# mfouda/epsilon

Measured on AMD Instinct MI355X. Metric: ADMM iters/sec, dense Lasso 1e4x5e4, higher is better.
Workload: dtype f32

## Files before the change

epsilon_amd/csrc/kernels_factor.hip:

```cpp
#include <hip/hip_runtime.h>

#include <algorithm>
#include <cstdlib>
#include <type_traits>

#include "kernels.h"
#include "options.h"

namespace eps {
namespace k {

namespace {

constexpr int NB = 64;

template <int L> __device__ inline float ReadLane(float v) {
  return __builtin_bit_cast(float, __builtin_amdgcn_readlane(__builtin_bit_cast(int, v), L));
}
template <int L> __device__ inline double ReadLane(double v) {
  const long long b = __builtin_bit_cast(long long, v);
  const int lo = __builtin_amdgcn_readlane(static_cast<int>(b), L);
  const int hi = __builtin_amdgcn_readlane(static_cast<int>(b >> 32), L);
  return __builtin_bit_cast(double, (static_cast<long long>(hi) << 32) |
                                        static_cast<unsigned int>(lo));
}

template <int I, int N> struct StaticFor {
  template <class F> __device__ static inline void Run(F&& f) {
    f(std::integral_constant<int, I>());
    StaticFor<I + 1, N>::Run(f);
  }
};
template <int N> struct StaticFor<N, N> {
  template <class F> __device__ static inline void Run(F&&) {}
};

constexpr int KC = 32;

template <class T> __device__ inline void Pin(T& v) { asm volatile("" : "+v"(v)); }

template <class T> __device__ __forceinline__ bool CholRows(T (&r)[NB], int lane) {
  bool bad = false;
  StaticFor<0, NB>::Run([&](auto jj) {
    constexpr int j = decltype(jj)::value;
    T d = ReadLane<j>(r[j]);
    if (!(d > T(0))) {
      bad = true;
      d = T(1);
    }
    const T dj = sqrt(d);
    const T l = lane > j ? r[j] / dj : (lane == j ? dj : T(0));
    r[j] = l;
    StaticFor<0, (NB - 1 - j + 3) / 4>::Run([&](auto gg) {
      constexpr int c0 = j + 1 + 4 * decltype(gg)::value;
      T b[4];
      StaticFor<0, 4>::Run([&](auto ii) {
        constexpr int c = c0 + decltype(ii)::value;
        if constexpr (c < NB) b[decltype(ii)::value] = ReadLane<c>(l);
      });
      StaticFor<0, 4>::Run([&](auto ii) {
        constexpr int c = c0 + decltype(ii)::value;
        if constexpr (c < NB) r[c] -= l * b[decltype(ii)::value];
      });
      StaticFor<0, 4>::Run([&](auto ii) {
        constexpr int c = c0 + decltype(ii)::value;
        if constexpr (c < NB) Pin(r[c]);
      });
    });
  });
  return bad;
}

template <class T> __device__ __forceinline__ bool CholRowsSolve(T (&r)[NB], T (&t)[NB], int lane) {
  bool bad = false;
  StaticFor<0, NB>::Run([&](auto jj) {
    constexpr int j = decltype(jj)::value;
    T d = ReadLane<j>(r[j]);
    if (!(d > T(0))) {
      bad = true;
      d = T(1);
    }
    const T dj = sqrt(d);
    const T l = lane > j ? r[j] / dj : (lane == j ? dj : T(0));
    r[j] = l;
    const T x = t[j] / dj;
    t[j] = x;
    StaticFor<0, (NB - 1 - j + 3) / 4>::Run([&](auto gg) {
      constexpr int c0 = j + 1 + 4 * decltype(gg)::value;
      T b[4];
      StaticFor<0, 4>::Run([&](auto ii) {
        constexpr int c = c0 + decltype(ii)::value;
        if constexpr (c < NB) b[decltype(ii)::value] = ReadLane<c>(l);
      });
      StaticFor<0, 4>::Run([&](auto ii) {
        constexpr int c = c0 + decltype(ii)::value;
        if constexpr (c < NB) {
          r[c] -= l * b[decltype(ii)::value];
          t[c] -= x * b[decltype(ii)::value];
        }
      });
      StaticFor<0, 4>::Run([&](auto ii) {
        constexpr int c = c0 + decltype(ii)::value;
        if constexpr (c < NB) {
          Pin(r[c]);
          Pin(t[c]);
        }
      });
    });
  });
  return bad;
}

template <class T>
__global__ __launch_bounds__(256) void PotrfDiagStepKernel(T* W, int64_t ld, int64_t K0, int64_t k0,
                                                           int kb, int* flag) {
  __shared__ T D[NB][NB];
  __shared__ T Pc[KC][NB];
  const int t = threadIdx.x, r = t & 63, q = t >> 6;
  T acc[16];
#pragma unroll
  for (int c = 0; c < 16; ++c) {
    const int col = q * 16 + c;
    T v = (r == col) ? T(1) : T(0);
    if (r < kb && col < kb && r >= col) v = W[(k0 + r) + (k0 + col) * ld];
    acc[c] = v;
  }
  constexpr int PF = KC * NB / 256;
  T pf[PF];
  auto fetch = [&](int64_t kk) {
#pragma unroll
    for (int i = 0; i < PF; ++i) {
      const int idx = t + i * 256, rr = idx & 63, k = idx >> 6;
      pf[i] = rr < kb ? W[(k0 + rr) + (kk + k) * ld] : T(0);
    }
  };
  if (K0 < k0) fetch(K0);
  for (int64_t kk = K0; kk < k0; kk += KC) {
    __syncthreads();
#pragma unroll
    for (int i = 0; i < PF; ++i) {
      const int idx = t + i * 256;
      Pc[idx >> 6][idx & 63] = pf[i];
    }
    __syncthreads();
    if (kk + KC < k0) fetch(kk + KC);
#pragma unroll 4
    for (int k = 0; k < KC; ++k) {
      const T a = Pc[k][r];
#pragma unroll
      for (int c = 0; c < 16; ++c) acc[c] -= a * Pc[k][q * 16 + c];
    }
  }
#pragma unroll
  for (int c = 0; c < 16; ++c) D[q * 16 + c][r] = acc[c];
  __syncthreads();
  if (q != 0) return;
  T row[NB];
  StaticFor<0, NB>::Run([&](auto cc) {
    constexpr int c = decltype(cc)::value;
    row[c] = r >= c ? D[c][r] : T(0);
  });
  const bool bad = CholRows(row, r);
  if (bad && r == 0) *flag = 1;
  StaticFor<0, NB>::Run([&](auto cc) {
    constexpr int c = decltype(cc)::value;
    if (r < kb && c < kb && r >= c) W[(k0 + r) + (k0 + c) * ld] = row[c];
  });
}

template <class T>
__global__ __launch_bounds__(256) void PotrfPanelStepKernel(T* W, int64_t ld, int64_t n, int64_t K0,
                                                            int64_t k0, int kb) {
  __shared__ T Tt[NB][NB];
  __shared__ T buf[2 * KC * NB];
  T* Lr = buf;
  T* Pc = buf + KC * NB;
  const int t = threadIdx.x, r = t & 63, q = t >> 6;
  const int64_t row0 = k0 + kb + static_cast<int64_t>(blockIdx.x) * NB;
  const int64_t row = row0 + r;
  const bool live = row < n;
  T acc[16];
#pragma unroll
  for (int c = 0; c < 16; ++c) {
    const int col = q * 16 + c;
    acc[c] = (live && col < kb) ? W[row + (k0 + col) * ld] : T(0);
  }
  constexpr int PF = KC * NB / 256;
  T pfl[PF], pfp[PF];
  auto fetch = [&](int64_t kk) {
#pragma unroll
    for (int i = 0; i < PF; ++i) {
      const int idx = t + i * 256, rr = idx & 63, k = idx >> 6;
      pfl[i] = (row0 + rr < n) ? W[(row0 + rr) + (kk + k) * ld] : T(0);
      pfp[i] = rr < kb ? W[(k0 + rr) + (kk + k) * ld] : T(0);
    }
  };
  if (K0 < k0) fetch(K0);
  for (int64_t kk = K0; kk < k0; kk += KC) {
    __syncthreads();
#pragma unroll
    for (int i = 0; i < PF; ++i) {
      const int idx = t + i * 256;
      Lr[idx] = pfl[i];
      Pc[idx] = pfp[i];
    }
    __syncthreads();
    if (kk + KC < k0) fetch(kk + KC);
#pragma unroll 4
    for (int k = 0; k < KC; ++k) {
      const T a = Lr[k * NB + r];
#pragma unroll
      for (int c = 0; c < 16; ++c) acc[c] -= a * Pc[k * NB + q * 16 + c];
    }
  }
  __syncthreads();
#pragma unroll
  for (int c = 0; c < 16; ++c) Tt[q * 16 + c][r] = acc[c];
  for (int idx = t; idx < NB * NB; idx += 256) {
    const int j = idx & 63, k = idx >> 6;
    T v = (j == k) ? T(1) : T(0);
    if (j < kb && k < kb && j >= k) v = W[(k0 + j) + (k0 + k) * ld];
    buf[j * NB + k] = v;
  }
  __syncthreads();
  if (q == 0) {
#pragma unroll 1
    for (int jb = 0; jb < NB; jb += 8) {
      T tv[8];
#pragma unroll
      for (int jj = 0; jj < 8; ++jj) tv[jj] = Tt[jb + jj][r];
#pragma unroll 1
      for (int k8 = 0; k8 < jb; k8 += 8) {
#pragma unroll
        for (int kk = 0; kk < 8; ++kk) {
          const T xk = Tt[k8 + kk][r];
#pragma unroll
          for (int jj = 0; jj < 8; ++jj) tv[jj] -= xk * buf[(jb + jj) * NB + k8 + kk];
        }
      }
#pragma unroll
      for (int jj = 0; jj < 8; ++jj) {
#pragma unroll
        for (int kk = 0; kk < jj; ++kk) tv[jj] -= tv[kk] * buf[(jb + jj) * NB + jb + kk];
        tv[jj] /= buf[(jb + jj) * NB + jb + jj];
      }
#pragma unroll
      for (int jj = 0; jj < 8; ++jj) Tt[jb + jj][r] = tv[jj];
    }
  }
  __syncthreads();
  if (live) {
#pragma unroll
    for (int c = 0; c < 16; ++c) {
      const int col = q * 16 + c;
      if (col < kb) W[row + (k0 + col) * ld] = Tt[col][r];
    }
  }
}

__global__ __launch_bounds__(256) void PotrfFusedStepKernel(float* W, int64_t ld, int64_t n, int64_t K0,
                                                            int64_t k0, int kb, int* flag,
                                                            float* __restrict__ dfac) {
  using T = float;
  __shared__ T Tt[NB][NB];
  __shared__ T Dd[NB][NB];
  __shared__ T buf[2 * KC * NB];
  T* Lr = buf;
  T* Pc = buf + KC * NB;
  const int t = threadIdx.x, r = t & 63, q = t >> 6;
  const int64_t row0 = k0 + kb + static_cast<int64_t>(blockIdx.x) * NB;
  const int64_t row = row0 + r;
  const bool live = row < n;
  T acc[16], dac[16];
#pragma unroll
  for (int c = 0; c < 16; ++c) {
    const int col = q * 16 + c;
    acc[c] = (live && col < kb) ? W[row + (k0 + col) * ld] : T(0);
    T v = (r == col) ? T(1) : T(0);
    if (r < kb && col < kb && r >= col) v = W[(k0 + r) + (k0 + col) * ld];
    dac[c] = v;
  }
  constexpr int PF = KC * NB / 256;
  T pfl[PF], pfp[PF];
  auto fetch = [&](int64_t kk) {
#pragma unroll
    for (int i = 0; i < PF; ++i) {
      const int idx = t + i * 256, rr = idx & 63, k = idx >> 6;
      pfl[i] = (row0 + rr < n) ? W[(row0 + rr) + (kk + k) * ld] : T(0);
      pfp[i] = rr < kb ? W[(k0 + rr) + (kk + k) * ld] : T(0);
    }
  };
  if (K0 < k0) fetch(K0);
  for (int64_t kk = K0; kk < k0; kk += KC) {
    __syncthreads();
#pragma unroll
    for (int i = 0; i < PF; ++i) {
      const int idx = t + i * 256;
      Lr[idx] = pfl[i];
      Pc[idx] = pfp[i];
    }
    __syncthreads();
    if (kk + KC < k0) fetch(kk + KC);
#pragma unroll 4
    for (int k = 0; k < KC; ++k) {
      const T a = Lr[k * NB + r], d = Pc[k * NB + r];
#pragma unroll
      for (int c = 0; c < 16; ++c) {
        const T pc = Pc[k * NB + q * 16 + c];
        acc[c] -= a * pc;
        dac[c] -= d * pc;
      }
    }
  }
  __syncthreads();
#pragma unroll
  for (int c = 0; c < 16; ++c) {
    Tt[q * 16 + c][r] = acc[c];
    Dd[q * 16 + c][r] = dac[c];
  }
  __syncthreads();
  if (q == 0) {
    T rowv[NB], tv[NB];
    StaticFor<0, NB>::Run([&](auto cc) {
      constexpr int c = decltype(cc)::value;
      rowv[c] = r >= c ? Dd[c][r] : T(0);
      tv[c] = Tt[c][r];
    });
    const bool bad = CholRowsSolve(rowv, tv, r);
    if (bad && r == 0) *flag = 1;
    StaticFor<0, NB>::Run([&](auto cc) {
      constexpr int c = decltype(cc)::value;
      Tt[c][r] = tv[c];
      if (blockIdx.x == 0) dfac[c * NB + r] = rowv[c];
    });
  }
  __syncthreads();
  if (live) {
#pragma unroll
    for (int c = 0; c < 16; ++c) {
      const int col = q * 16 + c;
      if (col < kb) W[row + (k0 + col) * ld] = Tt[col][r];
    }
  }
}

template <class T>
__global__ __launch_bounds__(64) void TrtriDiagBlocksKernel(const T* W, int64_t ld, int64_t n, T* Dinv) {
  const int lane = threadIdx.x;
  const int64_t k0 = static_cast<int64_t>(blockIdx.x) * NB;
  const int kb = static_cast<int>(n - k0 < NB ? n - k0 : NB);
  T r[NB];
  StaticFor<0, NB>::Run([&](auto cc) {
    constexpr int c = decltype(cc)::value;
    T v = (lane == c) ? T(1) : T(0);
    if (lane < kb && c < kb && lane >= c) v = W[(k0 + lane) + (k0 + c) * ld];
    r[c] = v;
  });
  T x[NB];
  StaticFor<0, NB>::Run([&](auto ii) {
    constexpr int j = NB - 1 - decltype(ii)::value;
    const T ajj = T(1) / ReadLane<j>(r[j]);
    T acc = T(0);
    StaticFor<0, (NB - 1 - j + 3) / 4>::Run([&](auto gg) {
      constexpr int c0 = j + 1 + 4 * decltype(gg)::value;
      T b[4];
      StaticFor<0, 4>::Run([&](auto ii) {
        constexpr int kk = c0 + decltype(ii)::value;
        if constexpr (kk < NB) b[decltype(ii)::value] = ReadLane<kk>(r[j]);
      });
      StaticFor<0, 4>::Run([&](auto ii) {
        constexpr int kk = c0 + decltype(ii)::value;
        if constexpr (kk < NB) acc += x[kk] * b[decltype(ii)::value];
      });
      Pin(acc);
    });
    x[j] = lane > j ? -acc * ajj : (lane == j ? ajj : T(0));
  });
  T* out = Dinv + static_cast<int64_t>(blockIdx.x) * NB * NB;
  StaticFor<0, NB>::Run([&](auto cc) {
    constexpr int c = decltype(cc)::value;
    out[lane + c * NB] = (lane < kb && c < kb && lane >= c) ? x[c] : T(0);
  });
}

template <class T>
__global__ __launch_bounds__(256) void ScatterDiagBlocksKernel(const T* Dinv, T* X, int64_t ld, int64_t n) {
  const int64_t k0 = static_cast<int64_t>(blockIdx.x) * NB;
  const T* src = Dinv + static_cast<int64_t>(blockIdx.x) * NB * NB;
  for (int idx = threadIdx.x; idx < NB * NB; idx += 256) {
    const int r = idx & 63, c = idx >> 6;
    if (k0 + r < n && k0 + c < n) X[(k0 + r) + (k0 + c) * ld] = src[idx];
  }
}

DVec Sub(const DVec& W, int64_t i, int64_t j, int64_t ld) {
  const int64_t off = i + j * ld;
  return W.Slice(off, W.n - off);
}

}

namespace {
void PotrfBlocked(const DVec& W, int64_t n, const DVec& dinv, int* flag);
void CheckFlag(int* flag);
void DoublingInverse(const DVec& W, const DVec& X, int64_t n, const DVec& dinv, int64_t cap);
}

void SpdInverseInPlace(const DVec& W, int64_t n, DVec* factor_inverse) {
  EPS_CHECK(W.n >= n * n);
  if (n == 0) return;
  Runtime& rt = Runtime::Get();
  hipStream_t s = rt.stream();
  ProfScope prof("spd_inverse", n);
  const DType dt = W.dt;
  const int64_t ld = n;
  const int64_t nb = (n + NB - 1) / NB;

  DVec dinv = DVec::Empty(nb * NB * NB, dt);
  auto flag_buf = rt.Alloc(sizeof(int));
  int* flag = static_cast<int*>(flag_buf->p);
  EPS_HIP(hipMemsetAsync(flag, 0, sizeof(int), s));
  {
    ProfScope p1("potrf", n);
    PotrfBlocked(W, n, dinv, flag);
  }

  DVec X = DVec::Zeros(n * n, dt);
  {
    ProfScope p2("trtri", n);
    DoublingInverse(W, X, n, dinv, n);
  }
  ProfScope p3("lauum", n);

  if (!SyrkSplitF16LowerTriangular(n, X, ld, W, ld)) {
    const int64_t B = 1024;
    Fill(W.Slice(0, n * n), 0.0);
    for (int64_t p0 = 0; p0 < n; p0 += B) {
      const int64_t pb = std::min<int64_t>(B, n - p0);
      const int64_t cp = p0 + pb;
      DVec Xp = Sub(X, p0, 0, ld);
      Gemm(true, false, cp, cp, pb, 1.0, Xp, ld, Xp, ld, 1.0, W, ld, true);
    }
  }
  SymmetrizeFromLower(W, n, ld);

  CheckFlag(flag);
  if (factor_inverse) *factor_inverse = X;
}

namespace {

void CheckFlag(int* flag) {
  hipStream_t s = Runtime::Get().stream();
  int host_flag = 0;
  EPS_HIP(hipMemcpyAsync(&host_flag, flag, sizeof(int), hipMemcpyDeviceToHost, s));
  EPS_HIP(hipStreamSynchronize(s));
  EPS_CHECK_MSG(host_flag == 0, "dense inverse: matrix is not positive definite");
}

void DoublingInverse(const DVec& W, const DVec& X, int64_t n, const DVec& dinv, int64_t cap) {
  hipStream_t s = Runtime::Get().stream();
  const DType dt = W.dt;
  const int64_t ld = n;
  const int64_t nb = (n + NB - 1) / NB;
  if (dt == F32)
    hipLaunchKernelGGL(ScatterDiagBlocksKernel<float>, dim3(static_cast<unsigned>(nb)), dim3(256), 0, s,
                       dinv.as<float>(), X.as<float>(), ld, n);
  else
    hipLaunchKernelGGL(ScatterDiagBlocksKernel<double>, dim3(static_cast<unsigned>(nb)), dim3(256), 0, s,
                       dinv.as<double>(), X.as<double>(), ld, n);
  const int64_t half = std::min<int64_t>(cap, n) / 2 + NB;
  const int64_t kBatchBelow = 4096;
  DVec tmp2 = DVec::Empty(std::max<int64_t>({1, half * half, n * std::min(cap, kBatchBelow) / 4}), dt);
  for (int64_t sz = NB; sz < cap; sz *= 2) {
    int64_t r_first = 0;
    if (sz < kBatchBelow) {
      const int64_t P = n / (2 * sz);
      if (P > 0) {
        const int64_t stride = 2 * sz * (ld + 1);
        EPS_CHECK(tmp2.n >= P * sz * sz);
        GemmBatched(false, false, sz, sz, sz, 1.0, Sub(W, sz, 0, ld), ld, stride, X, ld, stride, 0.0,
                    tmp2, sz, sz * sz, P);
        GemmBatched(false, false, sz, sz, sz, -1.0, Sub(X, sz, sz, ld), ld, stride, tmp2, sz, sz * sz,
                    0.0, Sub(X, sz, 0, ld), ld, stride, P);
      }
      r_first = P * 2 * sz;
    }
    for (int64_t r0 = r_first; r0 + sz < n; r0 += 2 * sz) {
      const int64_t s1 = sz;
      const int64_t s2 = std::min<int64_t>(sz, n - (r0 + sz));
      DVec L21 = Sub(W, r0 + s1, r0, ld);
      DVec X11 = Sub(X, r0, r0, ld);
      DVec X22 = Sub(X, r0 + s1, r0 + s1, ld);
      DVec X21 = Sub(X, r0 + s1, r0, ld);
      EPS_CHECK(tmp2.n >= s2 * s1);
      DVec T = tmp2.Slice(0, s2 * s1);
      const int64_t tiles = ((s1 + 127) / 128) * ((s2 + 127) / 128);
      const int64_t nsplit = std::max<int64_t>(1, std::min<int64_t>(4, tiles / 400));
      const int64_t cb = (s1 + nsplit - 1) / nsplit;
      const bool t_done = GemmSplitF16KRange(3, s2, s1, s1, 1.0, L21, ld, X11, ld, T, s2);
      for (int64_t c0 = 0; c0 < s1 && !t_done; c0 += cb) {
        const int64_t cw = std::min<int64_t>(cb, s1 - c0);
        Gemm(false, false, s2, cw, s1 - c0, 1.0, Sub(L21, 0, c0, ld), ld, Sub(X11, c0, c0, ld), ld,
             0.0, T.Slice(c0 * s2, cw * s2), s2);
      }
      const int64_t rb = (s2 + nsplit - 1) / nsplit;
      const bool x_done = GemmSplitF16KRange(4, s2, s1, s2, -1.0, X22, ld, T, s2, X21, ld);
      for (int64_t r1 = 0; r1 < s2 && !x_done; r1 += rb) {
        const int64_t rw = std::min<int64_t>(rb, s2 - r1);
        Gemm(false, false, rw, s1, r1 + rw, -1.0, Sub(X22, r1, 0, ld), ld, T, s2, 0.0,
             Sub(X21, r1, 0, ld), ld);
      }
    }
  }

}

int g_potrf_form = -1;

void PotrfBlocked(const DVec& W, int64_t n, const DVec& dinv, int* flag) {
  Runtime& rt = Runtime::Get();
  hipStream_t s = rt.stream();
  const DType dt = W.dt;
  const int64_t ld = n;
  const int64_t OB = 4 * NB;
  {
    const bool two_kernels = g_potrf_form == 1 ||
                             (g_potrf_form < 0 && opt::IsSet(opt::kPotrfTwoKernels));
    const unsigned nblk = static_cast<unsigned>((n + NB - 1) / NB);
    const bool fused = dt == F32 && !two_kernels;
    std::shared_ptr<Buffer> dfac_buf;
    if (fused) dfac_buf = rt.Alloc(static_cast<size_t>(nblk) * NB * NB * sizeof(float));
    float* dfac = fused ? static_cast<float*>(dfac_buf->p) : nullptr;
    for (int64_t K0 = 0; K0 < n; K0 += OB) {
      const int64_t KB = std::min<int64_t>(OB, n - K0);
      for (int64_t k0 = K0; k0 < K0 + KB; k0 += NB) {
        const int kb = static_cast<int>(std::min<int64_t>(NB, n - k0));
        const int64_t rem = n - (k0 + kb);
        const unsigned blocks = static_cast<unsigned>((rem + NB - 1) / NB);
        if (dt == F32) {
          if (fused) {
            hipLaunchKernelGGL(PotrfFusedStepKernel, dim3(blocks ? blocks : 1), dim3(256), 0, s,
                               W.as<float>(), ld, n, K0, k0, kb, flag, dfac + (k0 / NB) * NB * NB);
          } else {
            hipLaunchKernelGGL(PotrfDiagStepKernel<float>, dim3(1), dim3(256), 0, s, W.as<float>(), ld,
                               K0, k0, kb, flag);
            if (blocks)
              hipLaunchKernelGGL(PotrfPanelStepKernel<float>, dim3(blocks), dim3(256), 0, s,
                                 W.as<float>(), ld, n, K0, k0, kb);
          }
        } else {
          hipLaunchKernelGGL(PotrfDiagStepKernel<double>, dim3(1), dim3(256), 0, s, W.as<double>(),
                             ld, K0, k0, kb, flag);
          if (blocks)
            hipLaunchKernelGGL(PotrfPanelStepKernel<double>, dim3(blocks), dim3(256), 0, s,
                               W.as<double>(), ld, n, K0, k0, kb);
        }
      }
      const int64_t rem2 = n - (K0 + KB);
      if (rem2 > 0) {
        DVec L21 = Sub(W, K0 + KB, K0, ld);
        DVec W22 = Sub(W, K0 + KB, K0 + KB, ld);
        Gemm(false, true, rem2, rem2, KB, -1.0, L21, ld, L21, ld, 1.0, W22, ld, true);
      }
    }
    if (fused)
      hipLaunchKernelGGL(ScatterDiagBlocksKernel<float>, dim3(nblk), dim3(256), 0, s, dfac, W.as<float>(), ld, n);
    if (dt == F32)
      hipLaunchKernelGGL(TrtriDiagBlocksKernel<float>, dim3(nblk), dim3(64), 0, s, W.as<float>(), ld, n,
                         dinv.as<float>());
    else
      hipLaunchKernelGGL(TrtriDiagBlocksKernel<double>, dim3(nblk), dim3(64), 0, s, W.as<double>(), ld,
                         n, dinv.as<double>());
  }
}

}

void SetPotrfForm(int form) { g_potrf_form = form; }

void SpdInverseColumns(const DVec& W, int64_t n, int64_t lo, int64_t cnt, const DVec& Out) {
  EPS_CHECK(W.n >= n * n && Out.n >= n * cnt && Out.dt == W.dt && lo >= 0 && lo + cnt <= n);
  if (n == 0) return;
  Runtime& rt = Runtime::Get();
  hipStream_t s = rt.stream();
  ProfScope prof("spd_inverse_columns", n, cnt);
  const DType dt = W.dt;
  const int64_t ld = n;
  const int64_t nb = (n + NB - 1) / NB;
  DVec dinv = DVec::Empty(nb * NB * NB, dt);
  auto flag_buf = rt.Alloc(sizeof(int));
  int* flag = static_cast<int*>(flag_buf->p);
  EPS_HIP(hipMemsetAsync(flag, 0, sizeof(int), s));
  PotrfBlocked(W, n, dinv, flag);
  if (cnt == 0) {
    CheckFlag(flag);
    return;
  }
  Fill(Out.Slice(0, n * cnt), 0.0);
  AddDiag(Sub(Out, lo, 0, ld), cnt, ld, 1.0, nullptr);
  const int64_t BS = 512;
  DVec X = DVec::Zeros(n * n, dt);
  DoublingInverse(W, X, n, dinv, BS);
  DVec tmp = DVec::Empty(BS * cnt, dt);
  const size_t es = DTypeSize(dt);
  const int64_t nbs = (n + BS - 1) / BS;
  auto store_rows = [&](int64_t k0, int64_t kb) {
    EPS_HIP(hipMemcpy2DAsync(Sub(Out, k0, 0, ld).data(), ld * es, tmp.data(), kb * es, kb * es, cnt,
                             hipMemcpyDeviceToDevice, s));
  };
  for (int64_t kblk = lo / BS; kblk < nbs; ++kblk) {
    const int64_t k0 = kblk * BS;
    const int64_t kb = std::min<int64_t>(BS, n - k0);
    Gemm(false, false, kb, cnt, kb, 1.0, Sub(X, k0, k0, ld), ld, Sub(Out, k0, 0, ld), ld, 0.0, tmp,
         kb);
    store_rows(k0, kb);
    const int64_t rem = n - (k0 + kb);
    if (rem > 0)
      Gemm(false, false, rem, cnt, kb, -1.0, Sub(W, k0 + kb, k0, ld), ld, tmp, kb, 1.0,
           Sub(Out, k0 + kb, 0, ld), ld);
  }
  for (int64_t kblk = nbs - 1; kblk >= 0; --kblk) {
    const int64_t k0 = kblk * BS;
    const int64_t kb = std::min<int64_t>(BS, n - k0);
    Gemm(true, false, kb, cnt, kb, 1.0, Sub(X, k0, k0, ld), ld, Sub(Out, k0, 0, ld), ld, 0.0, tmp,
         kb);
    store_rows(k0, kb);
    if (k0 > 0)
      Gemm(true, false, k0, cnt, kb, -1.0, Sub(W, k0, 0, ld), ld, tmp, kb, 1.0, Out, ld);
  }
  CheckFlag(flag);
}

}
}
```

Before: 3378.

## Use MFMA for fused potrf trailing update and split diagonal solve across waves

The fused Cholesky step kernel now does its rank-k trailing update with 32x32x2 f32 MFMA instructions instead of scalar FMAs, and uses a larger K chunk (KCF=64). The 64-column diagonal factor-and-solve, which a single wave used to run, is split into four 16-column panels. Each wave factors its own panel and the other waves apply its update through shared memory, so all four waves work. Reciprocal square roots use a refined rsq with a sqrt fallback for tiny pivots. The changes add more barriers, shared-memory traffic and register pressure, and make small numeric differences possible.

After: 3390 (median of 3 runs). About the same (+0.3%).

```diff
diff --git a/epsilon_amd/csrc/kernels_factor.hip b/epsilon_amd/csrc/kernels_factor.hip
--- a/epsilon_amd/csrc/kernels_factor.hip
+++ b/epsilon_amd/csrc/kernels_factor.hip
@@ -71,46 +71,6 @@
   return bad;
 }
 
-template <class T> __device__ __forceinline__ bool CholRowsSolve(T (&r)[NB], T (&t)[NB], int lane) {
-  bool bad = false;
-  StaticFor<0, NB>::Run([&](auto jj) {
-    constexpr int j = decltype(jj)::value;
-    T d = ReadLane<j>(r[j]);
-    if (!(d > T(0))) {
-      bad = true;
-      d = T(1);
-    }
-    const T dj = sqrt(d);
-    const T l = lane > j ? r[j] / dj : (lane == j ? dj : T(0));
-    r[j] = l;
-    const T x = t[j] / dj;
-    t[j] = x;
-    StaticFor<0, (NB - 1 - j + 3) / 4>::Run([&](auto gg) {
-      constexpr int c0 = j + 1 + 4 * decltype(gg)::value;
-      T b[4];
-      StaticFor<0, 4>::Run([&](auto ii) {
-        constexpr int c = c0 + decltype(ii)::value;
-        if constexpr (c < NB) b[decltype(ii)::value] = ReadLane<c>(l);
-      });
-      StaticFor<0, 4>::Run([&](auto ii) {
-        constexpr int c = c0 + decltype(ii)::value;
-        if constexpr (c < NB) {
-          r[c] -= l * b[decltype(ii)::value];
-          t[c] -= x * b[decltype(ii)::value];
-        }
-      });
-      StaticFor<0, 4>::Run([&](auto ii) {
-        constexpr int c = c0 + decltype(ii)::value;
-        if constexpr (c < NB) {
-          Pin(r[c]);
-          Pin(t[c]);
-        }
-      });
-    });
-  });
-  return bad;
-}
-
 template <class T>
 __global__ __launch_bounds__(256) void PotrfDiagStepKernel(T* W, int64_t ld, int64_t K0, int64_t k0,
                                                            int kb, int* flag) {
@@ -258,89 +218,174 @@
   }
 }
 
+typedef float V2f __attribute__((ext_vector_type(2)));
+typedef float V4f __attribute__((ext_vector_type(4)));
+typedef float V16f __attribute__((ext_vector_type(16)));
+
+constexpr int MB = 16;
+constexpr int KCF = 64;
+
+__device__ __forceinline__ void PivotRoot(float d, float* dj, float* rinv) {
+  if (d >= 0x1p-96f) {
+    const float y0 = __builtin_amdgcn_rsqf(d);
+    const float s0 = d * y0;
+    const float s1 = fmaf(fmaf(-s0, s0, d), 0.5f * y0, s0);
+    *dj = s1;
+    *rinv = fmaf(fmaf(-s1, y0, 1.0f), y0, y0);
+  } else {
+    Pin(d);
+    const float s = sqrt(d);
+    *dj = s;
+    *rinv = 1.0f / s;
+  }
+}
+
 __global__ __launch_bounds__(256) void PotrfFusedStepKernel(float* W, int64_t ld, int64_t n, int64_t K0,
                                                             int64_t k0, int kb, int* flag,
                                                             float* __restrict__ dfac) {
   using T = float;
   __shared__ T Tt[NB][NB];
   __shared__ T Dd[NB][NB];
-  __shared__ T buf[2 * KC * NB];
+  __shared__ __attribute__((aligned(16))) T buf[2 * KCF * NB];
   T* Lr = buf;
-  T* Pc = buf + KC * NB;
-  const int t = threadIdx.x, r = t & 63, q = t >> 6;
+  T* Pc = buf + KCF * NB;
+  const int t = threadIdx.x, r = t & 63;
+  const int q = __builtin_amdgcn_readfirstlane(t >> 6);
   const int64_t row0 = k0 + kb + static_cast<int64_t>(blockIdx.x) * NB;
+  {
+    const int lr = r & 31, lh = r >> 5, rh = q >> 1, ch = q & 1;
+    const int rt = 32 * rh + lr;
+    const bool live_t = row0 + rt < n;
+    V16f ct, cd;
+#pragma unroll
+    for (int v = 0; v < 16; ++v) {
+      const int col = 32 * ch + 8 * (v >> 2) + 4 * lh + (v & 3);
+      ct[v] = (live_t && col < kb) ? W[(row0 + rt) + (k0 + col) * ld] : T(0);
+      T d = (rt == col) ? T(1) : T(0);
+      if (rt < kb && col < kb && rt >= col) d = W[(k0 + rt) + (k0 + col) * ld];
+      cd[v] = d;
+    }
+    constexpr int PF = KCF * NB / 256;
+    T pfl[PF], pfp[PF];
+    auto fetch = [&](int64_t kk) {
+#pragma unroll
+      for (int i = 0; i < PF; ++i) {
+        const int idx = t + i * 256, rr = idx & 63, k = idx >> 6;
+        pfl[i] = (row0 + rr < n) ? W[(row0 + rr) + (kk + k) * ld] : T(0);
+        pfp[i] = rr < kb ? W[(k0 + rr) + (kk + k) * ld] : T(0);
+      }
+    };
+    if (K0 < k0) fetch(K0);
+    for (int64_t kk = K0; kk < k0; kk += KCF) {
+      __syncthreads();
+#pragma unroll
+      for (int i = 0; i < PF; ++i) {
+        const int idx = t + i * 256;
+        Lr[idx] = pfl[i];
+        Pc[idx] = pfp[i];
+      }
+      __syncthreads();
+      if (kk + KCF < k0) fetch(kk + KCF);
+#pragma unroll 8
+      for (int k2 = 0; k2 < KCF; k2 += 2) {
+        const T a = -Pc[(k2 + lh) * NB + 32 * ch + lr];
+        const T bt = Lr[(k2 + lh) * NB + rt];
+        const T bd = Pc[(k2 + lh) * NB + rt];
+        ct = __builtin_amdgcn_mfma_f32_32x32x2f32(a, bt, ct, 0, 0, 0);
+        cd = __builtin_amdgcn_mfma_f32_32x32x2f32(a, bd, cd, 0, 0, 0);
+      }
+    }
+    __syncthreads();
+#pragma unroll
+    for (int v = 0; v < 16; ++v) {
+      const int col = 32 * ch + 8 * (v >> 2) + 4 * lh + (v & 3);
+      Tt[col][rt] = ct[v];
+      Dd[col][rt] = cd[v];
+    }
+    __syncthreads();
+  }
+  V2f p[MB];
+#pragma unroll
+  for (int c = 0; c < MB; ++c) {
+    const int col = MB * q + c;
+    const T d = Dd[col][r];
+    p[c].x = r >= col ? d : T(0);
+    p[c].y = Tt[col][r];
+  }
+  bool bad = false;
+  StaticFor<0, NB / MB>::Run([&](auto mm) {
+    constexpr int m = decltype(mm)::value;
+    T* Lp = buf + (m & 1) * 2 * MB * NB;
+    T* Xp = Lp + MB * NB;
+    if (q == m) {
+      StaticFor<0, MB>::Run([&](auto jj) {
+        constexpr int j = decltype(jj)::value;
+        constexpr int J = MB * m + j;
+        T d = ReadLane<J>(p[j].x);
+        if (!(d > T(0))) {
+          bad = true;
+          d = T(1);
+        }
+        T dj, rinv;
+        PivotRoot(d, &dj, &rinv);
+        const T l = r > J ? p[j].x * rinv : (r == J ? dj : T(0));
+        V2f lx;
+        lx.x = l;
+        lx.y = p[j].y * rinv;
+        p[j] = lx;
+        StaticFor<0, (MB - 1 - j + 3) / 4>::Run([&](auto gg) {
+          constexpr int c0 = j + 1 + 4 * decltype(gg)::value;
+          T b[4];
+          StaticFor<0, 4>::Run([&](auto ii) {
+            constexpr int c = c0 + decltype(ii)::value;
+            if constexpr (c < MB) b[decltype(ii)::value] = ReadLane<MB * m + c>(l);
+          });
+          StaticFor<0, 4>::Run([&](auto ii) {
+            constexpr int c = c0 + decltype(ii)::value;
+            if constexpr (c < MB) p[c] -= lx * b[decltype(ii)::value];
+          });
+          StaticFor<0, 4>::Run([&](auto ii) {
+            constexpr int c = c0 + decltype(ii)::value;
+            if constexpr (c < MB) Pin(p[c]);
+          });
+        });
+      });
+      if (bad && r == 0) *flag = 1;
+      if constexpr (m + 1 < NB / MB) {
+#pragma unroll
+        for (int j = 0; j < MB; ++j) {
+          Lp[j * NB + r] = p[j].x;
+          Xp[j * NB + r] = p[j].y;
+        }
+      }
+    }
+    if constexpr (m + 1 < NB / MB) {
+      __syncthreads();
+      if (q > m) {
+#pragma unroll
+        for (int k = 0; k < MB; ++k) {
+          V2f lx;
+          lx.x = Lp[k * NB + r];
+          lx.y = Xp[k * NB + r];
+#pragma unroll
+          for (int c4 = 0; c4 < MB; c4 += 4) {
+            const V4f b = *reinterpret_cast<const V4f*>(&Lp[k * NB + MB * q + c4]);
+            p[c4 + 0] -= lx * b.x;
+            p[c4 + 1] -= lx * b.y;
+            p[c4 + 2] -= lx * b.z;
+            p[c4 + 3] -= lx * b.w;
+          }
+        }
+      }
+    }
+  });
   const int64_t row = row0 + r;
   const bool live = row < n;
-  T acc[16], dac[16];
-#pragma unroll
-  for (int c = 0; c < 16; ++c) {
-    const int col = q * 16 + c;
-    acc[c] = (live && col < kb) ? W[row + (k0 + col) * ld] : T(0);
-    T v = (r == col) ? T(1) : T(0);
-    if (r < kb && col < kb && r >= col) v = W[(k0 + r) + (k0 + col) * ld];
-    dac[c] = v;
-  }
-  constexpr int PF = KC * NB / 256;
-  T pfl[PF], pfp[PF];
-  auto fetch = [&](int64_t kk) {
-#pragma unroll
-    for (int i = 0; i < PF; ++i) {
-      const int idx = t + i * 256, rr = idx & 63, k = idx >> 6;
-      pfl[i] = (row0 + rr < n) ? W[(row0 + rr) + (kk + k) * ld] : T(0);
-      pfp[i] = rr < kb ? W[(k0 + rr) + (kk + k) * ld] : T(0);
-    }
-  };
-  if (K0 < k0) fetch(K0);
-  for (int64_t kk = K0; kk < k0; kk += KC) {
-    __syncthreads();
-#pragma unroll
-    for (int i = 0; i < PF; ++i) {
-      const int idx = t + i * 256;
-      Lr[idx] = pfl[i];
-      Pc[idx] = pfp[i];
-    }
-    __syncthreads();
-    if (kk + KC < k0) fetch(kk + KC);
-#pragma unroll 4
-    for (int k = 0; k < KC; ++k) {
-      const T a = Lr[k * NB + r], d = Pc[k * NB + r];
-#pragma unroll
-      for (int c = 0; c < 16; ++c) {
-        const T pc = Pc[k * NB + q * 16 + c];
-        acc[c] -= a * pc;
-        dac[c] -= d * pc;
-      }
-    }
-  }
-  __syncthreads();
-#pragma unroll
-  for (int c = 0; c < 16; ++c) {
-    Tt[q * 16 + c][r] = acc[c];
-    Dd[q * 16 + c][r] = dac[c];
-  }
-  __syncthreads();
-  if (q == 0) {
-    T rowv[NB], tv[NB];
-    StaticFor<0, NB>::Run([&](auto cc) {
-      constexpr int c = decltype(cc)::value;
-      rowv[c] = r >= c ? Dd[c][r] : T(0);
-      tv[c] = Tt[c][r];
-    });
-    const bool bad = CholRowsSolve(rowv, tv, r);
-    if (bad && r == 0) *flag = 1;
-    StaticFor<0, NB>::Run([&](auto cc) {
-      constexpr int c = decltype(cc)::value;
-      Tt[c][r] = tv[c];
-      if (blockIdx.x == 0) dfac[c * NB + r] = rowv[c];
-    });
-  }
-  __syncthreads();
-  if (live) {
-#pragma unroll
-    for (int c = 0; c < 16; ++c) {
-      const int col = q * 16 + c;
-      if (col < kb) W[row + (k0 + col) * ld] = Tt[col][r];
-    }
+#pragma unroll
+  for (int c = 0; c < MB; ++c) {
+    const int col = MB * q + c;
+    if (blockIdx.x == 0) dfac[col * NB + r] = p[c].x;
+    if (live && col < kb) W[row + (k0 + col) * ld] = p[c].y;
   }
 }
 
```
